# HBioquant/DiffBindFR

Hardware: AMD Instinct MI355X
Metric: poses_per_sec (higher is better)
Workload: dtype f32

## Files before the change

diffbindfr_amd/csrc/api.cpp:

```cpp
#include <cmath>
#include <cstdio>
#include <cstring>
#include <algorithm>
#include <atomic>
#include <map>

#include "common.h"

void launch_conv(const ConvArgs& a, hipStream_t st);
void launch_conv_layer(const ConvArgs* c4, hipStream_t st);
void launch_conv2(const Conv2Args& a, hipStream_t st);
void launch_conv2h(const Conv2Args& a, hipStream_t st);
void launch_convz(const ConvZArgs& a, hipStream_t st);
void launch_reduce_ln(const float* msg, const int* row_start, const int* row_cnt, int N, int D, const LNDesc& ln,
                      const float* old, int D_old, float* out, int ldo, int mode, hipStream_t st, const uint8_t* first = nullptr, unsigned long long sc_lanes = 0);
struct ReduceLayerArgs {
  const float* msg[4]; const int* row_start[4]; const int* row_cnt[4]; LNDesc ln[4];
  int NL, NA, D, D_old;
  const float* old_l; const float* old_a; float* out_l; float* out_a;
  const uint8_t* first[4]; unsigned long long sc_lanes[4];
};
static unsigned long long convz_sc_lanes(const ConvZ& z) {
  unsigned long long m = 0;
  for (int i = 0; i < z.n_io; ++i) m |= 0xfffull << (z.out_off[i] / 4);
// ... 509 lines not shown
          const PathDesc* p = pidx >= 0 ? pairs[pidx].paths[pi] : lp;
          for (int r = 0; r < 4; ++r) {
            rows_orig.push_back(pidx >= 0 ? p->w_off + (u0 + r) * p->mulo + pairs[pidx].w : -1);
            rows_scale.push_back(pidx >= 0 ? p->fold : 0.f);
          }
        }
    }
  }
  const int n_tiles = (int)rows_orig.size() / 16;
  std::vector<float> w2q((size_t)n_tiles * KT * 64 * 4), b2q((size_t)n_tiles * 16);
  for (int t = 0; t < n_tiles; ++t) {
    for (int i = 0; i < 16; ++i) { const int ro = rows_orig[16 * t + i]; b2q[16 * t + i] = ro >= 0 ? rows_scale[16 * t + i] * B2[ro] : 0.f; }
    for (int s4 = 0; s4 < KT; ++s4)
      for (int lane = 0; lane < 64; ++lane) {
        const int ro = rows_orig[16 * t + (lane & 15)];
        const float sc = rows_scale[16 * t + (lane & 15)];
        for (int q = 0; q < 4; ++q)
          w2q[(((size_t)t * KT + s4) * 64 + lane) * 4 + q] = ro >= 0 ? sc * W2[(size_t)ro * K + 16 * s4 + 4 * (lane >> 4) + q] : 0.f;
      }
  }
  memset(o, 0, sizeof *o);
  o->D_in = sp.D_in; o->D_out = sp.D_out; o->n_tiles = n_tiles; o->n_runs = (int)runs.size();
  o->W1p = base.W1p; o->b1 = base.b1;
  if (!vector_only) {
  o->W2q = upload(m, w2q, &rc);
  o->b2q = upload(m, b2q, &rc);
  }
  {
    const int rowscale = getenv("DBFR_F16_ROWSCALE") ? atoi(getenv("DBFR_F16_ROWSCALE")) : 1;
    std::vector<uint16_t> w2h((size_t)n_tiles * (CH_TILE_BYTES_HOST / 2) + 512, 0);
    std::vector<float> w2rinv((size_t)std::max(n_tiles, 1) * 16, 1.f);
    int depth_max = 0, depth_run = 0;
    for (int pass = 0; pass < 2; ++pass) {
      const bool rowf = pass == 1;
      if (rowf && !(rowscale == 2 || (rowscale == 1 && depth_max > F16_ROW_DEPTH_OK))) break;
      if (rowf) depth_run = depth_max;
      depth_max = 0;
      for (RunDesc& rd : runs) {
        const int tile0 = rd.tile0_n & 0xfffff, nt = rd.tile0_n >> 20;
        int depth = 0;
        const int k = pack_f16_tiles(w2q.data(), b2q.data(), tile0, nt, w2h.data(), &depth, rowf ? w2rinv.data() : nullptr);
        depth_max = std::max(depth_max, depth);
        rd.meta = (rd.meta & 0x00ffffffu) | ((uint32_t)(k & 0xff) << 24);
      }
      if (!rowf) depth_run = depth_max;
      else o->W2rinv = upload(m, w2rinv, &rc);
    }
    o->W2h = upload(m, w2h, &rc);
    const float* W1 = need(tm, name + ".fc.lin.0.weight", (int64_t)K * K, &rc);
    const float* B1 = need(tm, name + ".fc.lin.0.bias", K, &rc);
    if (rc) return rc;
    std::vector<float> w1q((size_t)KT * KT * 256);
    for (int mt = 0; mt < KT; ++mt)
      for (int s4 = 0; s4 < KT; ++s4)
        for (int lane = 0; lane < 64; ++lane)
          for (int q = 0; q < 4; ++q)
            w1q[(((size_t)mt * KT + s4) * 64 + lane) * 4 + q] = W1[(size_t)(16 * mt + (lane & 15)) * K + 16 * s4 + 4 * (lane >> 4) + q];
    std::vector<uint16_t> w1h((size_t)KT * (CH_TILE_BYTES_HOST / 2) + 512, 0);
    int depth1 = 0;
    o->k1 = pack_f16_tiles(w1q.data(), B1, 0, KT, w1h.data(), &depth1);
    depth_run = std::max(depth_run, depth1);
    if (rowscale == 2 || (rowscale == 1 && depth1 > F16_ROW_DEPTH_OK)) {
      std::vector<float> w1rinv((size_t)KT * 16, 1.f);
      o->k1 = pack_f16_tiles(w1q.data(), B1, 0, KT, w1h.data(), &depth1, w1rinv.data());
      o->W1rinv = upload(m, w1rinv, &rc);
    }
    o->W1h = upload(m, w1h, &rc);
    o->f16_depth = std::max(depth_max, depth1);
    o->f16_depth_run = depth_run;
  }
  o->runs = upload(m, runs, &rc);
  const int n_g = (int)groups.size();
  int total_tiles = 0;
  for (int t : group_tiles) total_tiles += t;
  for (int si = 0; si < 4; ++si) {
    const int S = 1 << si;
    int gi = 0, acc = 0;
    for (int p = 0; p < S; ++p) {
      o->part_run[si][p] = gi < n_g ? group_run0[gi] : (int)runs.size();
      const long target = (long)total_tiles * (p + 1) / S;
      while (gi < n_g && (acc + group_tiles[gi] / 2 < target || p == S - 1)) { acc += group_tiles[gi]; ++gi; }
    }
    for (int p = S; p <= 8; ++p) o->part_run[si][p] = (int)runs.size();
  }
  return rc;
}

static int pack_convz(dbfr_model* m, const TMap& tm, const std::string& name, int kind, const ConvW2& base, ConvZ* o) {
  ConvSpec sp = make_conv_spec(kind);
  const int K = sp.K;
  memset(o, 0, sizeof *o);
  if (K != 144) return fail(DBFR_ERR_ARG, "k_convz is for the K=144 convs");
  int rc = 0;
  const float* W2 = need(tm, name + ".fc.lin.3.weight", (int64_t)sp.W * K, &rc);
  const float* B2 = need(tm, name + ".fc.lin.3.bias", sp.W, &rc);
  if (rc) return rc;
  struct Col { const PathDesc* p; int u; };
  std::vector<std::vector<Col>> cols;
  std::vector<int> ios;
  for (int io = 0; io < (int)sp.out.size(); ++io) {
    if (sp.out[io].l != 0) continue;
    if (sp.out[io].mul != NS) return fail(DBFR_ERR_ARG, "scalar output irrep with a multiplicity other than 48 in " + name);
    std::vector<Col> c;
    for (int pass = 0; pass < 2; ++pass)
      for (auto& p : sp.paths) {
        if (p.io != io || p.l1 != pass) continue;
        if (p.l1 != p.l2 || p.lo != 0 || p.l1 > 1) return fail(DBFR_ERR_ARG, "unsupported scalar-output path in " + name);
        for (int u = 0; u < p.mul1; ++u) c.push_back({&p, u});
      }
    int n_scalar = 0;
    for (auto& q : c) n_scalar += q.p->l1 == 0;
    if (n_scalar % 16) return fail(DBFR_ERR_ARG, "scalar-input columns do not fill whole tiles in " + name);
    while (c.size() % 16) c.push_back({nullptr, 0});
    cols.push_back(c);
    ios.push_back(io);
  }
  if (ios.size() > 2) return fail(DBFR_ERR_ARG, "more than two scalar output irreps in " + name);
  o->n_io = (int)ios.size();
  int nct_total = 0;
  for (int i = 0; i < o->n_io; ++i) {
    o->nct[i] = (int)cols[i].size() / 16;
    for (auto& q : cols[i]) o->nc_valid[i] += q.p != nullptr;
    o->ct0[i] = nct_total;
    nct_total += o->nct[i];
    int off = 0;
    for (int j = 0; j < ios[i]; ++j) off += sp.out[j].mul * sp.out[j].dim();
    o->out_off[i] = off;
  }
  if (nct_total > CZ_MAXCT) return fail(DBFR_ERR_ARG, "too many c tiles in " + name);
  std::vector<uint32_t> cdesc((size_t)std::max(nct_total, 1) * 16, 0u);
  std::vector<float> rowinv((size_t)std::max(o->n_io, 1) * NS, 1.f);
  std::vector<uint16_t> w2z((size_t)nct_total * CZ_NKT * 8 * (CZ_TILE_BYTES / 2) + 512, 0);
  auto h16 = [](float v) { const _Float16 h = (_Float16)v; uint16_t u; memcpy(&u, &h, 2); return u; };
  for (int i = 0; i < o->n_io; ++i) {
    const auto& c = cols[i];
    for (size_t j = 0; j < c.size(); ++j)
      if (c[j].p) cdesc[(size_t)o->ct0[i] * 16 + j] = (uint32_t)(c[j].p->in_off + c[j].u * (2 * c[j].p->l1 + 1)) | ((uint32_t)c[j].p->l1 << 12) |
                                                      ((uint32_t)c[j].p->sh_off << 16) | 0x80000000u;
    auto wval = [&](int cc, int k, int w) -> float {
      if (cc >= (int)c.size() || !c[cc].p || k > K) return 0.f;
      const PathDesc* p = c[cc].p;
      const size_t row = (size_t)p->w_off + (size_t)c[cc].u * p->mulo + w;
      return p->fold * (k < K ? W2[row * K + k] : B2[row]);
    };
    for (int w = 0; w < NS; ++w) {
      float mx = 0.f;
      for (int cc = 0; cc < (int)c.size(); ++cc)
        for (int k = 0; k <= K; ++k) mx = std::max(mx, fabsf(wval(cc, k, w)));
      int s = 0;
      if (mx > 0.f) { int e = 0; (void)frexpf(mx, &e); s = std::max(-100, std::min(100, 15 - e)); }
      rowinv[(size_t)i * NS + w] = ldexpf(1.f, -s);
      const float sc = ldexpf(1.f, s);
      const int wt = w >> 4, np = w & 15;
      for (int ct = 0; ct < o->nct[i]; ++ct)
        for (int kt = 0; kt < CZ_NKT; ++kt)
          for (int v = 0; v < 8; ++v)
            for (int gp = 0; gp < 4; ++gp)
              for (int t = 0; t < 8; ++t) {
                const float val = wval(16 * ct + 4 * gp + (t & 3), 16 * kt + v + 8 * (t >> 2), w) * sc;
                const _Float16 hi = (_Float16)val;
                const size_t tile = ((size_t)(o->ct0[i] + ct) * CZ_NKT + kt) * 8 + v;
                const size_t base_h = tile * (CZ_TILE_BYTES / 2) + (size_t)(wt * 2) * 512 + (size_t)(16 * gp + np) * 8 + t;
                w2z[base_h] = h16(val);
                w2z[base_h + 512] = h16(val - (float)hi);
              }
    }
// ... 967 lines not shown
```

diffbindfr_amd/csrc/common.h:

```cpp
#pragma once
#include <hip/hip_runtime.h>
#include <stdint.h>
#include <string.h>
#include <string>
#include <vector>

#include "../../include/dbfr.h"

#define NS 48
#define NV 12
#define SH_LD 9
#define EMB 32
#define MAXD 168
#define EDGE_CHUNK 64
int dbfr_edge_chunks(int max_na, int max_nl);

enum PathType { PT_SS = 0, PT_SV = 1, PT_VS = 2, PT_VVS = 3, PT_VVV = 4, PT_VTV = 5 };

struct Irr { int mul, l, p; int dim() const { return 2 * l + 1; } };

struct PathDesc {
  int i1, i2, io, l1, l2, lo, mul1, mulo, w_off;
  float coeff;
  int type;
  int in_off, sh_off, out_off;
  float fold;
};

struct ConvSpec {
  std::vector<Irr> in, sh, out;
  std::vector<PathDesc> paths;
  int K;
  int W;
  int D_in, D_out;
};

ConvSpec make_conv_spec(int kind);
void wigner3j_real(int l1, int l2, int l3, std::vector<double>& out);
int so3_selftest(std::string& err);

struct LNDesc {
  int nblk;
  int mul[4], dim[4], off[4], is0e[4];
  const float* mean_shift;
  const float* weight;
  const float* bias;
};

struct RunDesc {
  uint32_t tile0_n;
  uint32_t meta;
  uint32_t x_off4;
  uint32_t o_off4;
};

struct ConvW {
  int K, D_in, D_out, n_tiles, W;
  int wave_tile0[5];
  const float* W1p;
  const float* b1;
  const float* W2p;
  const float* b2p;
  const RunDesc* runs;
  int wave_run0[5];
  LNDesc ln;
};

struct ConvW2 {
  int D_in, D_out, n_tiles, n_runs;
  const float* W1p;
  const float* b1;
  const float* W2q;
  const float* b2q;
  const void* W1h;
  int k1;
  int f16_depth;
  int f16_depth_run;
  const float* W2rinv;
  const float* W1rinv;
  const void* W2h;
  const RunDesc* runs;
  int part_run[4][9];
};

struct Conv2Desc {
  const int* n_edges; int max_edges;
  const int* gth;
  const float* emb;
  const float* sh;
  const float* tab1; int ld1; const int* idx1;
  const float* tab2; int ld2; const int* idx2;
  const float* x; int ldx;
  ConvW2 w;
  float* msg;
};

struct Conv2Args {
  Conv2Desc c[4];
  int n_conv;
  int* queue;
  int run_barrier, no_split;
  int skew;
  unsigned long long* trace;
};
#define C2_TRACE_CAP 4096

#define CZ_NKT 10
#define CZ_MAXCT 12
#define CZ_MAXSEG 4
#define CZ_TILE_BYTES 6144
struct ConvZ {
  int n_io;
  int nct[2];
  int ct0[2];
  int out_off[2];
  int nc_valid[2];
  const uint32_t* cdesc;
  const void* W2z;
  const float* rowinv;
  const void* W1h; int k1;
  const float* W1rinv;
};
struct ConvZDesc {
  const int* n_edges; int max_edges;
  const int* tgt;
  const int* gth;
  const float* emb; const float* sh;
  const float* tab1; int ld1; const int* idx1;
  const float* tab2; int ld2; const int* idx2;
  const float* x; int ldx;
  ConvZ w;
  float* msg; int D_out;
  const int* chunk_es;
  const int* chunk_gl;
  const int* n_chunks;
  int max_chunks;
  const float* xmax;
};
struct ConvZArgs { ConvZDesc c[4]; int n_conv; float* dbg; double* executed; int dbg_sel; };

static inline uint16_t dbfr_bf16_rne(float x) {
  uint32_t u;
  memcpy(&u, &x, 4);
  u += 0x7fffu + ((u >> 16) & 1u);
  return (uint16_t)(u >> 16);
}
static inline float dbfr_bf16_to_f32(uint16_t b) {
  const uint32_t u = (uint32_t)b << 16;
  float f;
  memcpy(&f, &u, 4);
  return f;
}

struct Mlp2 {
  int in, hid, out;
  const float* w0t;
  const float* b0;
  const float* w1t;
  const float* b1;
};

struct EdgeSet {
  int cap;
  int* n_edges;
  int* tgt;
// ... 47 lines not shown
```

diffbindfr_amd/csrc/conv2h.hip:

```cpp
#include <cstdio>
#include <cstdlib>
#include <type_traits>

#include "common.h"

typedef float f32x4 __attribute__((ext_vector_type(4)));
typedef float f32x2 __attribute__((ext_vector_type(2)));
typedef _Float16 f16x8 __attribute__((ext_vector_type(8)));
typedef _Float16 f16x4 __attribute__((ext_vector_type(4)));
typedef _Float16 f16x2 __attribute__((ext_vector_type(2)));
typedef unsigned u32x4 __attribute__((ext_vector_type(4)));
typedef unsigned u32x2 __attribute__((ext_vector_type(2)));

#define CH_TILE_BYTES 9280
#define CH_TAIL_OFF 8192
#define CH_BIAS_OFF 9216
#define CH_RING_BYTES 10240

__device__ __forceinline__ void split2x2(float x0, float x1, unsigned& hi, unsigned& lo) {
  const f16x2 h = __builtin_convertvector((f32x2){x0, x1}, f16x2);
  const f16x2 l = __builtin_convertvector((f32x2){x0 - (float)h[0], x1 - (float)h[1]}, f16x2);
  hi = __builtin_bit_cast(unsigned, h);
  lo = __builtin_bit_cast(unsigned, l);
}

__device__ __forceinline__ void scale4(f32x4& o, const f32x4& v, float s) { o[0] = v[0] * s; o[1] = v[1] * s; o[2] = v[2] * s; o[3] = v[3] * s; }
__device__ __forceinline__ void sum4(f32x4& o, const f32x4& a, const f32x4& b) { o[0] = a[0] + b[0]; o[1] = a[1] + b[1]; o[2] = a[2] + b[2]; o[3] = a[3] + b[3]; }

#define C2_XLD 124
#define C2_WAVE_FLOATS (32 * C2_XLD + 32 * 10 + 32 * 8 + 32)

template <int NW, int ABL = 0>
__global__ __launch_bounds__(64 * NW, 2) void k_conv2h(Conv2Args a) {
  constexpr int K = 144, KT = 9;
  constexpr bool ROWF = (ABL & 1024) != 0;
  constexpr int EPB = 32 * NW;
  extern __shared__ __attribute__((aligned(16))) float lds[];
  const int tid = threadIdx.x, lane = tid & 63, wave = tid >> 6;
  const int n = lane & 15, g = lane >> 4;
  if (wave >= NW / 2) __builtin_amdgcn_s_setprio(1);
  const char* ring = reinterpret_cast<const char*>(lds);
  float* xs = lds + CH_RING_BYTES / 4 + wave * C2_WAVE_FLOATS;
  float* shs = xs + 32 * C2_XLD;
  float* ms = shs + 32 * 10;
  int* s_gth = reinterpret_cast<int*>(ms + 32 * 8);

  if (a.trace && blockIdx.x == 0 && tid == 0) { a.trace[0] = __builtin_readcyclecounter(); a.trace[1] = __builtin_amdgcn_s_memrealtime(); }
  int nb0 = 0, nb1 = 0, nb2 = 0, nb3 = 0;
  {
    auto blocks = [&](int c) { return c < a.n_conv ? (min(*a.c[c].n_edges, a.c[c].max_edges) + EPB - 1) / EPB : 0; };
    nb0 = blocks(0); nb1 = blocks(1); nb2 = blocks(2); nb3 = blocks(3);
  }
  const int N = nb0 + nb1 + nb2 + nb3;
  const int n_wg = gridDim.x;
  const int full = (N / n_wg) * n_wg, rem = N - full;
  int si = 0;
  if (rem > 0 && !a.no_split) {
    int best = 0x7fffffff;
#pragma unroll
    for (int c = 0; c < 4; ++c) {
      const int cost = (((rem << c) + n_wg - 1) / n_wg) * ((128 >> c) + 6);
      if (cost < best) { best = cost; si = c; }
    }
  }
  const int total = full + (rem << si);

  for (int it = 0;; ++it) {
    asm volatile("s_waitcnt vmcnt(0) lgkmcnt(0)" ::: "memory");
    __syncthreads();
    const int u = (int)blockIdx.x + it * n_wg;
    if (u >= total) break;
    int blk, part = 0, psi = 0;
    if (u < full) blk = u;
    else { const int v = u - full; blk = full + (v >> si); part = v & ((1 << si) - 1); psi = si; }
    int c = 0;
    if (blk >= nb0) { blk -= nb0; c = 1; if (blk >= nb1) { blk -= nb1; c = 2; if (blk >= nb2) { blk -= nb2; c = 3; } } }
    const Conv2Desc& d = a.c[c];
    const int E = min(*d.n_edges, d.max_edges);
    const int e0 = blk * EPB + 32 * wave;
    const int D_in = d.w.D_in, D_out = d.w.D_out;
    const int vW = lane * 16, vB = g * 16;
    const int wv = __builtin_amdgcn_readfirstlane(wave);
    const int r_begin = d.w.part_run[psi][part], r_end = d.w.part_run[psi][part + 1];
    int t_last = 0, t_first = 0;
    if (r_begin < r_end) {
      const RunDesc rl = d.w.runs[r_end - 1];
      t_last = (rl.tile0_n & 0xfffff) + (rl.tile0_n >> 20) - 1;
      t_first = d.w.runs[r_begin].tile0_n & 0xfffff;
    }
    const __amdgpu_buffer_rsrc_t rW = __builtin_amdgcn_make_buffer_rsrc((void*)d.w.W2h, 0, d.w.n_tiles * CH_TILE_BYTES, 0x00020000);
    const int shA = wv & 7, shB = wv % 6;
    const int offA = shA < 6 ? ((shA / 3) * 4 + shA % 3) * 1024 : CH_BIAS_OFF;
    const int offB = shB < 4 ? ((shB >> 1) * 4 + 3) * 1024 + (shB & 1) * 512 : CH_TAIL_OFF + (shB - 4) * 512;
    const int vA = (shA < 6 || lane < 4) ? lane * 16 : 0x40000000;
    char* ringw = const_cast<char*>(ring);
    u32x4 stgA = {0u, 0u, 0u, 0u};
    u32x2 stgB = {0u, 0u};
    auto fetchA = [&](int tile) { if (!(ABL & (4 | 16))) stgA = __builtin_bit_cast(u32x4, __builtin_amdgcn_raw_buffer_load_b128(rW, vA, ((ABL & 512) ? (tile & 7) : tile) * CH_TILE_BYTES + offA, 0)); };
    auto fetchB = [&](int tile) { if (!(ABL & (4 | 16))) stgB = __builtin_bit_cast(u32x2, __builtin_amdgcn_raw_buffer_load_b64(rW, lane * 8, ((ABL & 512) ? (tile & 7) : tile) * CH_TILE_BYTES + offB, 0)); };
    auto putA = [&] { if (!(ABL & (4 | 8))) *reinterpret_cast<u32x4*>(ringw + offA + vW) = stgA; };
    auto putB = [&] { if (!(ABL & (4 | 8))) *reinterpret_cast<u32x2*>(ringw + offB + lane * 8) = stgB; };
    using I0 = std::integral_constant<int, 0>; using I1 = std::integral_constant<int, 1>;
    using I2 = std::integral_constant<int, 2>; using I3 = std::integral_constant<int, 3>;
    if (r_begin < r_end) {
      fetchA(t_first); fetchB(t_first);
    }

    int ev[2], gthv[2];
    const float* r0[2]; const float* r1[2]; const float* r2[2];
#pragma unroll
    for (int b = 0; b < 2; ++b) {
      const int e = e0 + 16 * b + n;
      ev[b] = min(e, E - 1);
      gthv[b] = d.gth[ev[b]];
      r0[b] = d.emb + (size_t)ev[b] * NS;
      r1[b] = d.tab1 + (size_t)d.idx1[ev[b]] * d.ld1;
      r2[b] = d.tab2 + (size_t)d.idx2[ev[b]] * d.ld2;
    }
    if (g == 0) { s_gth[n] = gthv[0]; s_gth[16 + n] = gthv[1]; }
    if (lane < 32) {
      const int e = min(e0 + lane, E - 1);
      const float* sp = d.sh + (size_t)e * SH_LD;
      float s[9];
#pragma unroll
      for (int k = 0; k < 9; ++k) { s[k] = sp[k]; shs[lane * 10 + k] = s[k]; }
      const float r3 = 1.7320508075688772f;
      float* m = ms + lane * 8;
      m[0] = -s[6] - r3 * s[8]; m[1] = r3 * s[5]; m[2] = r3 * s[4]; m[3] = 2.f * s[6]; m[4] = r3 * s[7]; m[5] = -s[6] + r3 * s[8];
    }
    u32x4 Bh[2][2][4];
    u32x4 Btc[2];
    float se[2], ue[2];
    {
      const __amdgpu_buffer_rsrc_t rW1 = __builtin_amdgcn_make_buffer_rsrc((void*)d.w.W1h, 0, KT * CH_TILE_BYTES, 0x00020000);
      u32x4 Ah[2][2][4];
      u32x4 Atc[2];
      float sa[2];
      int ja[2];
#pragma unroll
      for (int b = 0; b < 2; ++b) {
        f32x4 Ba[KT];
        float amx = 0.f;
#pragma unroll
        for (int s4 = 0; s4 < KT; ++s4) {
          const float* src = s4 < 3 ? r0[b] : s4 < 6 ? r1[b] : r2[b];
          Ba[s4] = *reinterpret_cast<const f32x4*>(src + 16 * (s4 % 3) + 4 * g);
#pragma unroll
          for (int q = 0; q < 4; ++q) amx = fmaxf(amx, fabsf(Ba[s4][q]));
        }
        amx = fmaxf(amx, __shfl_xor(amx, 16));
        amx = fmaxf(amx, __shfl_xor(amx, 32));
        ja[b] = max(-14, __builtin_amdgcn_frexp_expf(amx));
        sa[b] = __builtin_amdgcn_ldexpf(1.f, 15 - ja[b]);
#pragma unroll
        for (int s4 = 0; s4 < KT; ++s4) {
          unsigned hi0, lo0, hi1, lo1;
          split2x2(Ba[s4][0] * sa[b], Ba[s4][1] * sa[b], hi0, lo0);
          split2x2(Ba[s4][2] * sa[b], Ba[s4][3] * sa[b], hi1, lo1);
          if (s4 < 8) {
            Ah[b][0][s4 >> 1][2 * (s4 & 1)] = hi0; Ah[b][0][s4 >> 1][2 * (s4 & 1) + 1] = hi1;
            Ah[b][1][s4 >> 1][2 * (s4 & 1)] = lo0; Ah[b][1][s4 >> 1][2 * (s4 & 1) + 1] = lo1;
          } else {
            Atc[b] = (u32x4){lo0, lo1, hi0, hi1};
          }
        }
      }
      constexpr int NST = KT * 4;
      u32x4 F[3][2];
      u32x4 Ft;
      f32x4 bb;
      auto ld_step = [&](int i, u32x4 (&f)[2]) {
#pragma unroll
        for (int p = 0; p < 2; ++p) f[p] = __builtin_bit_cast(u32x4, __builtin_amdgcn_raw_buffer_load_b128(rW1, vW, (i >> 2) * CH_TILE_BYTES + (p * 4 + (i & 3)) * 1024, 0));
      };
      auto ld_tail = [&](int m) {
        Ft = __builtin_bit_cast(u32x4, __builtin_amdgcn_raw_buffer_load_b128(rW1, vW, m * CH_TILE_BYTES + CH_TAIL_OFF, 0));
        bb = __builtin_bit_cast(f32x4, __builtin_amdgcn_raw_buffer_load_b128(rW1, vB, m * CH_TILE_BYTES + CH_BIAS_OFF, 0));
      };
      ld_step(0, F[0]); ld_step(1, F[1]); ld_tail(0);
      float H[2][KT][4];
      float mx[2] = {0.f, 0.f};
      const f32x4 zero = {0.f, 0.f, 0.f, 0.f};
#define AHB(b, p, s) __builtin_bit_cast(f16x8, Ah[b][p][s])
#define FW(i, p) __builtin_bit_cast(f16x8, F[(i) % 3][p])
#pragma unroll
      for (int m = 0; m < KT; ++m) {
        f32x4 aS[2], aB[2];
        scale4(aS[0], bb, sa[0]); scale4(aS[1], bb, sa[1]);
        aB[0] = zero; aB[1] = zero;
#pragma unroll
        for (int s = 0; s < 4; ++s) {
          const int i = m * 4 + s;
          aS[0] = __builtin_amdgcn_mfma_f32_16x16x32_f16(FW(i, 0), AHB(0, 1, s), aS[0], 0, 0, 0);
          aS[1] = __builtin_amdgcn_mfma_f32_16x16x32_f16(FW(i, 0), AHB(1, 1, s), aS[1], 0, 0, 0);
          aS[0] = __builtin_amdgcn_mfma_f32_16x16x32_f16(FW(i, 1), AHB(0, 0, s), aS[0], 0, 0, 0);
          aS[1] = __builtin_amdgcn_mfma_f32_16x16x32_f16(FW(i, 1), AHB(1, 0, s), aS[1], 0, 0, 0);
          aB[0] = __builtin_amdgcn_mfma_f32_16x16x32_f16(FW(i, 0), AHB(0, 0, s), aB[0], 0, 0, 0);
          aB[1] = __builtin_amdgcn_mfma_f32_16x16x32_f16(FW(i, 0), AHB(1, 0, s), aB[1], 0, 0, 0);
          __builtin_amdgcn_sched_barrier(0);
          if (i + 2 < NST) ld_step(i + 2, F[(i + 2) % 3]);
        }
        {
          const f16x8 fw = __builtin_bit_cast(f16x8, Ft);
          const f16x4 fh = __builtin_bit_cast(f16x4, (u32x2){Ft[0], Ft[1]});
          aS[0] = __builtin_amdgcn_mfma_f32_16x16x32_f16(fw, __builtin_bit_cast(f16x8, Atc[0]), aS[0], 0, 0, 0);
          aS[1] = __builtin_amdgcn_mfma_f32_16x16x32_f16(fw, __builtin_bit_cast(f16x8, Atc[1]), aS[1], 0, 0, 0);
          aB[0] = __builtin_amdgcn_mfma_f32_16x16x16f16(fh, __builtin_bit_cast(f16x4, (u32x2){Atc[0][2], Atc[0][3]}), aB[0], 0, 0, 0);
          aB[1] = __builtin_amdgcn_mfma_f32_16x16x16f16(fh, __builtin_bit_cast(f16x4, (u32x2){Atc[1][2], Atc[1][3]}), aB[1], 0, 0, 0);
          __builtin_amdgcn_sched_barrier(0);
          if (m + 1 < KT) ld_tail(m + 1);
        }
        f32x4 rv = {1.f, 1.f, 1.f, 1.f};
        if constexpr (ROWF) if (d.w.W1rinv) rv = *reinterpret_cast<const f32x4*>(d.w.W1rinv + 16 * m + 4 * g);
#pragma unroll
        for (int b = 0; b < 2; ++b)
#pragma unroll
          for (int r = 0; r < 4; ++r) { H[b][m][r] = fmaxf(aS[b][r] + aB[b][r], 0.f); if constexpr (ROWF) H[b][m][r] *= rv[r]; mx[b] = fmaxf(mx[b], H[b][m][r]); }
      }
#undef AHB
#undef FW
      const int k1 = d.w.k1;
#pragma unroll
      for (int b = 0; b < 2; ++b) {
        float m2 = fmaxf(mx[b], __shfl_xor(mx[b], 16));
        m2 = fmaxf(m2, __shfl_xor(m2, 32));
        const int j = __builtin_amdgcn_frexp_expf(m2);
        const int tot = max(-120, min(64, 15 - j + k1 + 15 - ja[b]));
        const float t = __builtin_amdgcn_ldexpf(1.f, tot - k1 - 15 + ja[b]);
        se[b] = __builtin_amdgcn_ldexpf(1.f, tot);
        ue[b] = __builtin_amdgcn_ldexpf(1.f, -tot);
#pragma unroll
        for (int m = 0; m < KT; ++m) {
          unsigned hi0, lo0, hi1, lo1;
          split2x2(H[b][m][0] * t, H[b][m][1] * t, hi0, lo0);
          split2x2(H[b][m][2] * t, H[b][m][3] * t, hi1, lo1);
          if (m < 8) {
            Bh[b][0][m >> 1][2 * (m & 1)] = hi0; Bh[b][0][m >> 1][2 * (m & 1) + 1] = hi1;
            Bh[b][1][m >> 1][2 * (m & 1)] = lo0; Bh[b][1][m >> 1][2 * (m & 1) + 1] = lo1;
          } else {
            Btc[b] = (u32x4){lo0, lo1, hi0, hi1};
          }
        }
      }
    }
    __builtin_amdgcn_wave_barrier();
    {
      const int d4 = min(D_in, 120) >> 2;
      const float* xsrc = d.x + (size_t)s_gth[lane & 31] * d.ldx;
      float* xdst = xs + (lane & 31) * C2_XLD;
      f32x4 v[15];
#pragma unroll
      for (int j = 0; j < 15; ++j) v[j] = *reinterpret_cast<const f32x4*>(xsrc + 4 * min(2 * j + (lane >> 5), d4 - 1));
#pragma unroll
      for (int j = 0; j < 15; ++j) *reinterpret_cast<f32x4*>(xdst + 4 * min(2 * j + (lane >> 5), d4 - 1)) = v[j];
    }
    __builtin_amdgcn_wave_barrier();

    if (ABL & 64) {
      asm volatile("" ::"v"(Bh[0][0][0]), "v"(Bh[1][1][3]), "v"(Btc[1]));
      continue;
    }
    float oacc[2][3];
#pragma unroll
    for (int b = 0; b < 2; ++b) oacc[b][0] = oacc[b][1] = oacc[b][2] = 0.f;
    const float* xs_lane = xs + n * C2_XLD;
    const float* sh_lane = shs + n * 10;
    f16x8 FA[2], FB[2];
    f16x8 FT;
    f32x4 bias_n;
    f32x4 accN[2];
    f32x4 accS[2], accB[2];
    f32x4 accp[2];
    f32x4 rinv_c = {1.f, 1.f, 1.f, 1.f}, rinv_n = {1.f, 1.f, 1.f, 1.f};
    const float* rinv_base = ROWF && d.w.W2rinv ? d.w.W2rinv + 4 * g : nullptr;
    auto sumr4 = [&](f32x4& o, const f32x4& x, const f32x4& y) {
      if constexpr (ROWF) { o[0] = (x[0] + y[0]) * rinv_c[0]; o[1] = (x[1] + y[1]) * rinv_c[1]; o[2] = (x[2] + y[2]) * rinv_c[2]; o[3] = (x[3] + y[3]) * rinv_c[3]; }
      else sum4(o, x, y);
    };
    auto rd_step = [&](auto jc, f16x8 (&F)[2]) {
      constexpr int j = decltype(jc)::value;
#pragma unroll
      for (int i = 0; i < 2; ++i) F[i] = *reinterpret_cast<const f16x8*>(ring + (i * 4 + j) * 1024 + vW);
    };
    auto ring_barrier = [&] {
      __builtin_amdgcn_sched_barrier(0);
      asm volatile("s_waitcnt lgkmcnt(0)" ::: "memory");
      if (!(ABL & 2)) __builtin_amdgcn_s_barrier();
      __builtin_amdgcn_sched_barrier(0);
    };
#define HB(b, p, s) __builtin_bit_cast(f16x8, Bh[b][p][s])
#define M32(C, wp, b, hp, F, s) __builtin_amdgcn_mfma_f32_16x16x32_f16(F[wp], HB(b, hp, s), C, 0, 0, 0)
#define MT32(C, b) __builtin_amdgcn_mfma_f32_16x16x32_f16(FT, __builtin_bit_cast(f16x8, Btc[b]), C, 0, 0, 0)
#define MT16(C, b) __builtin_amdgcn_mfma_f32_16x16x16f16(__builtin_shufflevector(FT, FT, 0, 1, 2, 3), __builtin_bit_cast(f16x4, (u32x2){Btc[b][2], Btc[b][3]}), C, 0, 0, 0)
#define SLOT(m) do { op(std::integral_constant<int, (m)>{}); __builtin_amdgcn_sched_barrier(0); } while (0)
    auto tile = [&](int t, auto&& op) {
      const f32x4 zero = {0.f, 0.f, 0.f, 0.f};
      accS[0] = M32(accN[0], 0, 0, 1, FA, 0); if (ABL & 256) putB(); SLOT(0);
      accS[1] = M32(accN[1], 0, 1, 1, FA, 0); if (ABL & 256) fetchB(min(t + 1, t_last)); SLOT(1);
      accS[0] = M32(accS[0], 1, 0, 0, FA, 0); rd_step(I1{}, FB); SLOT(2);
      accS[1] = M32(accS[1], 1, 1, 0, FA, 0); SLOT(3);
      accB[0] = M32(zero, 0, 0, 0, FA, 0); SLOT(4);
      accB[1] = M32(zero, 0, 1, 0, FA, 0); SLOT(5);
      accS[0] = M32(accS[0], 0, 0, 1, FB, 1); SLOT(6);
      accS[1] = M32(accS[1], 0, 1, 1, FB, 1); SLOT(7);
      accS[0] = M32(accS[0], 1, 0, 0, FB, 1); rd_step(I2{}, FA); SLOT(8);
      accS[1] = M32(accS[1], 1, 1, 0, FB, 1); if (!(ABL & 256)) putB(); SLOT(9);
      accB[0] = M32(accB[0], 0, 0, 0, FB, 1); if (!(ABL & (256 | 32))) fetchB(min(t + 1, t_last)); SLOT(10);
      accB[1] = M32(accB[1], 0, 1, 0, FB, 1); SLOT(11);
      ring_barrier();
      accS[0] = M32(accS[0], 0, 0, 1, FA, 2); if (ABL & 256) putA(); SLOT(12);
      accS[1] = M32(accS[1], 0, 1, 1, FA, 2); if (ABL & 256) fetchA(min(t + 2, t_last)); SLOT(13);
      accS[0] = M32(accS[0], 1, 0, 0, FA, 2); rd_step(I3{}, FB); SLOT(14);
      accS[1] = M32(accS[1], 1, 1, 0, FA, 2); SLOT(15);
      accB[0] = M32(accB[0], 0, 0, 0, FA, 2); SLOT(16);
      accB[1] = M32(accB[1], 0, 1, 0, FA, 2); SLOT(17);
      accS[0] = M32(accS[0], 0, 0, 1, FB, 3); SLOT(18);
      accS[1] = M32(accS[1], 0, 1, 1, FB, 3); SLOT(19);
      accS[0] = M32(accS[0], 1, 0, 0, FB, 3); FT = *reinterpret_cast<const f16x8*>(ring + CH_TAIL_OFF + vW);
      if constexpr (ROWF) if (rinv_base) rinv_n = *reinterpret_cast<const f32x4*>(rinv_base + 16 * min(t + 1, t_last));
      SLOT(20);
      accS[1] = M32(accS[1], 1, 1, 0, FB, 3); if (!(ABL & 256)) putA(); SLOT(21);
      accB[0] = M32(accB[0], 0, 0, 0, FB, 3); if (!(ABL & (256 | 32))) fetchA(min(t + 2, t_last)); SLOT(22);
      accB[1] = M32(accB[1], 0, 1, 0, FB, 3); SLOT(23);
      ring_barrier();
      accS[0] = MT32(accS[0], 0); bias_n = *reinterpret_cast<const f32x4*>(ring + CH_BIAS_OFF + vB); SLOT(24);
      accB[0] = MT16(accB[0], 0); rd_step(I0{}, FA); SLOT(25);
      accS[1] = MT32(accS[1], 1); SLOT(26);
      accB[1] = MT16(accB[1], 1); SLOT(27);
      sumr4(accp[1], accS[1], accB[1]);
      if constexpr (ROWF) rinv_c = rinv_n;
      __builtin_amdgcn_sched_barrier(0);
    };
#undef SLOT
    int x_phase = 0;
    if (r_begin < r_end) {
      putA();
      fetchA(min(t_first + 1, t_last));
      asm volatile("s_waitcnt lgkmcnt(0)" ::: "memory");
      __builtin_amdgcn_s_barrier();
      rd_step(I0{}, FA);
      bias_n = *reinterpret_cast<const f32x4*>(ring + CH_BIAS_OFF + vB);
      scale4(accN[0], bias_n, se[0]); scale4(accN[1], bias_n, se[1]);
      if constexpr (ROWF) if (rinv_base) rinv_c = *reinterpret_cast<const f32x4*>(rinv_base + 16 * t_first);
    }
    for (int r = r_begin; r < r_end; ++r) {
      const RunDesc rd = d.w.runs[r];
      const int tile0 = rd.tile0_n & 0xfffff, nt = rd.tile0_n >> 20;
      const int type = rd.meta & 15, flags = (rd.meta >> 4) & 3, sh_off = (rd.meta >> 8) & 15, x_step = (rd.meta >> 12) & 0xff;
      const int xph = (rd.meta >> 20) & 1;
      const float run_inv = __builtin_amdgcn_ldexpf(1.f, -((int)rd.meta >> 24));
      const int xo = (rd.x_off4 >> (8 * g)) & 0xff, oo = (rd.o_off4 >> (8 * g)) & 0xff;
      if (xph != x_phase) {
        __builtin_amdgcn_wave_barrier();
        {
          const float* xsrc = d.x + (size_t)s_gth[lane & 31] * d.ldx + 120;
          float* xdst = xs + (lane & 31) * C2_XLD;
          f32x4 v[6];
#pragma unroll
          for (int j = 0; j < 6; ++j) v[j] = *reinterpret_cast<const f32x4*>(xsrc + 4 * (2 * j + (lane >> 5)));
#pragma unroll
          for (int j = 0; j < 6; ++j) *reinterpret_cast<f32x4*>(xdst + 4 * (2 * j + (lane >> 5))) = v[j];
        }
        __builtin_amdgcn_wave_barrier();
        x_phase = xph;
      }
      if (flags & 1) {
#pragma unroll
        for (int b = 0; b < 2; ++b) oacc[b][0] = oacc[b][1] = oacc[b][2] = 0.f;
      }
      auto run = [&](auto type_c) {
        constexpr int TYPE = decltype(type_c)::value;
        constexpr bool VIN = !(TYPE == PT_SS || TYPE == PT_SV);
        constexpr bool VOUT = !(TYPE == PT_SS || TYPE == PT_VVS);
        constexpr int NSV = (TYPE == PT_SS || TYPE == PT_VS) ? 1 : (TYPE == PT_VTV ? 0 : 3);
        float S[2][NSV ? NSV : 1];
        float Mv[2][TYPE == PT_VTV ? 6 : 1];
#pragma unroll
        for (int b = 0; b < 2; ++b) {
          if (TYPE != PT_VTV) {
            const float* sp = sh_lane + 160 * b + sh_off;
#pragma unroll
            for (int k = 0; k < NSV; ++k) S[b][k] = sp[k] * run_inv;
          } else {
            const float* mp = ms + (16 * b + n) * 8;
#pragma unroll
            for (int k = 0; k < 6; ++k) Mv[b][k] = mp[k] * run_inv;
          }
        }
        f32x4 cxa, cxb, cxc;
        float czr[2][3] = {{0.f, 0.f, 0.f}, {0.f, 0.f, 0.f}};
        auto cop = [&](auto bc, auto kc, const float* xp) {
          constexpr int b = decltype(bc)::value;
          constexpr int K = decltype(kc)::value;
          if (ABL & 1) { if (K == 1) asm volatile("" ::"v"(accp[b])); return; }
          const f32x4 v = accp[b];
          const f32x4* x4 = reinterpret_cast<const f32x4*>(xp + 16 * b * C2_XLD);
          if (VIN && K == 2) cxb = x4[1];
          if (VIN && K == 6) cxc = x4[2];
          if (K == 0) cxa = x4[0];
          if (!VIN) {
            if (K == 1) czr[b][0] += v[0] * cxa[0];
            if (K == 2) czr[b][0] += v[1] * cxa[1];
            if (K == 3) czr[b][0] += v[2] * cxa[2];
            if (K == 4) czr[b][0] += v[3] * cxa[3];
          } else {
            if (K == 1) czr[b][0] += v[0] * cxa[0];
            if (K == 2) czr[b][1] += v[0] * cxa[1];
            if (K == 3) czr[b][2] += v[0] * cxa[2];
            if (K == 4) czr[b][0] += v[1] * cxa[3];
            if (K == 5) czr[b][1] += v[1] * cxb[0];
            if (K == 6) czr[b][2] += v[1] * cxb[1];
            if (K == 7) czr[b][0] += v[2] * cxb[2];
            if (K == 8) czr[b][1] += v[2] * cxb[3];
            if (K == 9) czr[b][2] += v[2] * cxc[0];
            if (K == 10) czr[b][0] += v[3] * cxc[1];
            if (K == 11) czr[b][1] += v[3] * cxc[2];
            if (K == 12) czr[b][2] += v[3] * cxc[3];
          }
        };
        auto finish = [&](auto bc) {
          constexpr int b = decltype(bc)::value;
          if (ABL & 1) return;
          const float cz0 = czr[b][0], cz1 = czr[b][1], cz2 = czr[b][2];
          if (TYPE == PT_SS) oacc[b][0] += cz0 * S[b][0];
          else if (TYPE == PT_SV) { oacc[b][0] += cz0 * S[b][0]; oacc[b][1] += cz0 * S[b][1]; oacc[b][2] += cz0 * S[b][2]; }
          else if (TYPE == PT_VS) { oacc[b][0] += cz0 * S[b][0]; oacc[b][1] += cz1 * S[b][0]; oacc[b][2] += cz2 * S[b][0]; }
          else if (TYPE == PT_VVS) { oacc[b][0] += cz0 * S[b][0]; oacc[b][0] += cz1 * S[b][1]; oacc[b][0] += cz2 * S[b][2]; }
          else if (TYPE == PT_VVV) {
            oacc[b][0] += cz1 * S[b][2]; oacc[b][1] += cz2 * S[b][0]; oacc[b][2] += cz0 * S[b][1];
            oacc[b][0] -= cz2 * S[b][1]; oacc[b][1] -= cz0 * S[b][2]; oacc[b][2] -= cz1 * S[b][0];
          } else {
            oacc[b][0] += Mv[b][0] * cz0; oacc[b][1] += Mv[b][1] * cz0; oacc[b][2] += Mv[b][2] * cz0;
            oacc[b][0] += Mv[b][1] * cz1; oacc[b][1] += Mv[b][3] * cz1; oacc[b][2] += Mv[b][4] * cz1;
            oacc[b][0] += Mv[b][2] * cz2; oacc[b][1] += Mv[b][4] * cz2; oacc[b][2] += Mv[b][5] * cz2;
          }
        };
        using B0 = std::integral_constant<int, 0>;
        using B1 = std::integral_constant<int, 1>;
        auto travel = [&](auto mc, const float* xp) {
          constexpr int m = decltype(mc)::value;
          if constexpr (m == 0) cop(B0{}, std::integral_constant<int, 0>{}, xp);
          if constexpr (m >= 3 && m <= 14) cop(B0{}, std::integral_constant<int, m - 2>{}, xp);
          if constexpr (m == 12) cop(B1{}, std::integral_constant<int, 0>{}, xp);
          if constexpr (m >= 15 && m <= 26) cop(B1{}, std::integral_constant<int, m - 14>{}, xp);
          if constexpr (m == 26) scale4(accN[0], bias_n, se[0]);
          if constexpr (m == 27) { scale4(accN[1], bias_n, se[1]); sumr4(accp[0], accS[0], accB[0]); }
        };
        const float* xp = xs_lane + xo;
        accp[0] = (f32x4){0.f, 0.f, 0.f, 0.f}; accp[1] = (f32x4){0.f, 0.f, 0.f, 0.f};
        for (int i = 0; i < nt; ++i) {
          tile(tile0 + i, [&](auto mc) { travel(mc, xp); });
          if (i) xp += x_step;
        }
        __builtin_amdgcn_sched_barrier(0);
#define COPS(b) cop(b, std::integral_constant<int, 0>{}, xp); cop(b, std::integral_constant<int, 1>{}, xp); cop(b, std::integral_constant<int, 2>{}, xp); \
        cop(b, std::integral_constant<int, 3>{}, xp); cop(b, std::integral_constant<int, 4>{}, xp); cop(b, std::integral_constant<int, 5>{}, xp); \
        cop(b, std::integral_constant<int, 6>{}, xp); cop(b, std::integral_constant<int, 7>{}, xp); cop(b, std::integral_constant<int, 8>{}, xp); \
        cop(b, std::integral_constant<int, 9>{}, xp); cop(b, std::integral_constant<int, 10>{}, xp); cop(b, std::integral_constant<int, 11>{}, xp); \
        cop(b, std::integral_constant<int, 12>{}, xp); finish(b);
        COPS(B0{}) COPS(B1{})
#undef COPS
        if (flags & 2) {
          if (oo < D_out) {
#pragma unroll
            for (int b = 0; b < 2; ++b)
              if (e0 + 16 * b + n < E) {
                float* op = d.msg + (size_t)(e0 + 16 * b + n) * D_out + oo;
                op[0] = oacc[b][0] * ue[b];
                if (VOUT) { op[1] = oacc[b][1] * ue[b]; op[2] = oacc[b][2] * ue[b]; }
              }
          }
        }
      };
      switch (type) {
        case PT_SS: run(std::integral_constant<int, PT_SS>{}); break;
        case PT_SV: run(std::integral_constant<int, PT_SV>{}); break;
        case PT_VS: run(std::integral_constant<int, PT_VS>{}); break;
        case PT_VVS: run(std::integral_constant<int, PT_VVS>{}); break;
        case PT_VVV: run(std::integral_constant<int, PT_VVV>{}); break;
        default: run(std::integral_constant<int, PT_VTV>{}); break;
      }
    }
#undef M32
#undef MT32
#undef MT16
#undef HB
#undef TB
  }
  if (a.trace && blockIdx.x == 0 && tid == 0) { a.trace[2] = __builtin_readcyclecounter(); a.trace[3] = __builtin_amdgcn_s_memrealtime(); }
}

void launch_conv2h(const Conv2Args& a, hipStream_t st) {
  static int no_split = getenv("DBFR_CONV2_NOSPLIT") ? atoi(getenv("DBFR_CONV2_NOSPLIT")) : 0;
  constexpr int NW = 8;
  const size_t lds = CH_RING_BYTES + (size_t)NW * C2_WAVE_FLOATS * sizeof(float);
  const int n_cu = dbfr_current_cu_count();
  Conv2Args b = a;
  b.skew = 0;
  b.run_barrier = 0;
  b.no_split = no_split;
#define V(x) { if (dbfr_launch_check(hipFuncSetAttribute(reinterpret_cast<const void*>(&k_conv2h<NW, x>), hipFuncAttributeMaxDynamicSharedMemorySize, (int)lds), "k_conv2h: hipFuncSetAttribute(MaxDynamicSharedMemorySize)")) return; \
               hipLaunchKernelGGL((k_conv2h<NW, x>), dim3(n_cu), dim3(64 * NW), lds, st, b); return; }
#ifdef DBFR_DEV_VARIANTS
  static int abl = getenv("DBFR_CONV2H_ABL") ? atoi(getenv("DBFR_CONV2H_ABL")) : 0;
  if (abl == 1) V(1) if (abl == 2) V(2) if (abl == 3) V(3) if (abl == 4) V(4) if (abl == 7) V(7) if (abl == 8) V(8) if (abl == 16) V(16)
  if (abl == 32) V(32) if (abl == 64) V(64) if (abl == 256) V(256) if (abl == 512) V(512)
#endif
  for (int i = 0; i < a.n_conv; ++i)
    if (a.c[i].w.W2rinv || a.c[i].w.W1rinv) V(1024)
  V(0)
#undef V
}
```

Baseline: 510.9.

## Hoist edge loads and W1 weight prefetch ahead of the first conv2h layer

Reorders the prologue of the conv2h kernel so that edge embeddings, tables and SH values are loaded early. The first W1 weight steps, bias, tail and row-inverse are prefetched before the tab1/tab2 gathers, giving the memory latency room to overlap. Per-part first and last tile indices are precomputed on the host into a new part_tile table, which avoids dependent loads of run descriptors. Edge counts are read once per block through readfirstlane. Register pressure rises from the larger prefetch arrays, and optional timing stamps are added behind a dev macro.

```diff
diff --git a/diffbindfr_amd/csrc/api.cpp b/diffbindfr_amd/csrc/api.cpp
--- a/diffbindfr_amd/csrc/api.cpp
+++ b/diffbindfr_amd/csrc/api.cpp
@@ -615,6 +615,13 @@
       while (gi < n_g && (acc + group_tiles[gi] / 2 < target || p == S - 1)) { acc += group_tiles[gi]; ++gi; }
     }
     for (int p = S; p <= 8; ++p) o->part_run[si][p] = (int)runs.size();
+    for (int p = 0; p < 8; ++p) {
+      const int r0 = o->part_run[si][p], r1 = o->part_run[si][p + 1];
+      if (r0 >= r1) continue;
+      const uint32_t t_first = runs[r0].tile0_n & 0xfffff, t_last = (runs[r1 - 1].tile0_n & 0xfffff) + (runs[r1 - 1].tile0_n >> 20) - 1;
+      if (t_last >= (1u << 16)) return fail(DBFR_ERR_ARG, "conv too large for the part tile table");
+      o->part_tile[si][p] = t_first | (t_last << 16);
+    }
   }
   return rc;
 }
diff --git a/diffbindfr_amd/csrc/common.h b/diffbindfr_amd/csrc/common.h
--- a/diffbindfr_amd/csrc/common.h
+++ b/diffbindfr_amd/csrc/common.h
@@ -81,6 +81,7 @@
   const void* W2h;
   const RunDesc* runs;
   int part_run[4][9];
+  uint32_t part_tile[4][8];
 };
 
 struct Conv2Desc {
diff --git a/diffbindfr_amd/csrc/conv2h.hip b/diffbindfr_amd/csrc/conv2h.hip
--- a/diffbindfr_amd/csrc/conv2h.hip
+++ b/diffbindfr_amd/csrc/conv2h.hip
@@ -27,6 +27,20 @@
 __device__ __forceinline__ void scale4(f32x4& o, const f32x4& v, float s) { o[0] = v[0] * s; o[1] = v[1] * s; o[2] = v[2] * s; o[3] = v[3] * s; }
 __device__ __forceinline__ void sum4(f32x4& o, const f32x4& a, const f32x4& b) { o[0] = a[0] + b[0]; o[1] = a[1] + b[1]; o[2] = a[2] + b[2]; o[3] = a[3] + b[3]; }
 
+#ifdef DBFR_DEV_VARIANTS
+#define C2H_STAMP(k) do { __builtin_amdgcn_sched_barrier(0); stamp[k] = __builtin_readcyclecounter(); __builtin_amdgcn_sched_barrier(0); } while (0)
+#define C2H_STAMPS_OUT() do { if (a.trace && blockIdx.x == 0 && tid == 0 && it < 64) { for (int k = 0; k < 4; ++k) a.trace[8 + 4 * it + k] = stamp[k]; } } while (0)
+#else
+#define C2H_STAMP(k) do { } while (0)
+#define C2H_STAMPS_OUT() do { } while (0)
+#endif
+
+#ifndef C2H_RING_DEPTH
+#define C2H_RING_DEPTH 2
+#endif
+#ifndef C2H_PIN
+#define C2H_PIN 0
+#endif
 #define C2_XLD 124
 #define C2_WAVE_FLOATS (32 * C2_XLD + 32 * 10 + 32 * 8 + 32)
 
@@ -46,11 +60,9 @@
   int* s_gth = reinterpret_cast<int*>(ms + 32 * 8);
 
   if (a.trace && blockIdx.x == 0 && tid == 0) { a.trace[0] = __builtin_readcyclecounter(); a.trace[1] = __builtin_amdgcn_s_memrealtime(); }
-  int nb0 = 0, nb1 = 0, nb2 = 0, nb3 = 0;
-  {
-    auto blocks = [&](int c) { return c < a.n_conv ? (min(*a.c[c].n_edges, a.c[c].max_edges) + EPB - 1) / EPB : 0; };
-    nb0 = blocks(0); nb1 = blocks(1); nb2 = blocks(2); nb3 = blocks(3);
-  }
+  auto edges = [&](int c) { return c < a.n_conv ? __builtin_amdgcn_readfirstlane(min(*a.c[c].n_edges, a.c[c].max_edges)) : 0; };
+  const int E0 = edges(0), E1 = edges(1), E2 = edges(2), E3 = edges(3);
+  const int nb0 = (E0 + EPB - 1) / EPB, nb1 = (E1 + EPB - 1) / EPB, nb2 = (E2 + EPB - 1) / EPB, nb3 = (E3 + EPB - 1) / EPB;
   const int N = nb0 + nb1 + nb2 + nb3;
   const int n_wg = gridDim.x;
   const int full = (N / n_wg) * n_wg, rem = N - full;
@@ -70,24 +82,26 @@
     __syncthreads();
     const int u = (int)blockIdx.x + it * n_wg;
     if (u >= total) break;
+#ifdef DBFR_DEV_VARIANTS
+    unsigned long long stamp[4] = {0ull, 0ull, 0ull, 0ull};
+#endif
+    C2H_STAMP(0);
     int blk, part = 0, psi = 0;
     if (u < full) blk = u;
     else { const int v = u - full; blk = full + (v >> si); part = v & ((1 << si) - 1); psi = si; }
     int c = 0;
     if (blk >= nb0) { blk -= nb0; c = 1; if (blk >= nb1) { blk -= nb1; c = 2; if (blk >= nb2) { blk -= nb2; c = 3; } } }
     const Conv2Desc& d = a.c[c];
-    const int E = min(*d.n_edges, d.max_edges);
+    int cs = c;
+    asm volatile("" : "+s"(cs));
+    const int E = cs == 0 ? E0 : cs == 1 ? E1 : cs == 2 ? E2 : E3;
     const int e0 = blk * EPB + 32 * wave;
     const int D_in = d.w.D_in, D_out = d.w.D_out;
     const int vW = lane * 16, vB = g * 16;
     const int wv = __builtin_amdgcn_readfirstlane(wave);
     const int r_begin = d.w.part_run[psi][part], r_end = d.w.part_run[psi][part + 1];
-    int t_last = 0, t_first = 0;
-    if (r_begin < r_end) {
-      const RunDesc rl = d.w.runs[r_end - 1];
-      t_last = (rl.tile0_n & 0xfffff) + (rl.tile0_n >> 20) - 1;
-      t_first = d.w.runs[r_begin].tile0_n & 0xfffff;
-    }
+    const unsigned pt = d.w.part_tile[psi][part];
+    const int t_first = pt & 0xffff, t_last = pt >> 16;
     const __amdgpu_buffer_rsrc_t rW = __builtin_amdgcn_make_buffer_rsrc((void*)d.w.W2h, 0, d.w.n_tiles * CH_TILE_BYTES, 0x00020000);
     const int shA = wv & 7, shB = wv % 6;
     const int offA = shA < 6 ? ((shA / 3) * 4 + shA % 3) * 1024 : CH_BIAS_OFF;
@@ -102,52 +116,83 @@
     auto putB = [&] { if (!(ABL & (4 | 8))) *reinterpret_cast<u32x2*>(ringw + offB + lane * 8) = stgB; };
     using I0 = std::integral_constant<int, 0>; using I1 = std::integral_constant<int, 1>;
     using I2 = std::integral_constant<int, 2>; using I3 = std::integral_constant<int, 3>;
-    if (r_begin < r_end) {
-      fetchA(t_first); fetchB(t_first);
-    }
-
-    int ev[2], gthv[2];
-    const float* r0[2]; const float* r1[2]; const float* r2[2];
+    int ev[2], gthv[2], i1v[2], i2v[2];
 #pragma unroll
     for (int b = 0; b < 2; ++b) {
       const int e = e0 + 16 * b + n;
       ev[b] = min(e, E - 1);
       gthv[b] = d.gth[ev[b]];
-      r0[b] = d.emb + (size_t)ev[b] * NS;
-      r1[b] = d.tab1 + (size_t)d.idx1[ev[b]] * d.ld1;
-      r2[b] = d.tab2 + (size_t)d.idx2[ev[b]] * d.ld2;
-    }
-    if (g == 0) { s_gth[n] = gthv[0]; s_gth[16 + n] = gthv[1]; }
-    if (lane < 32) {
-      const int e = min(e0 + lane, E - 1);
-      const float* sp = d.sh + (size_t)e * SH_LD;
-      float s[9];
-#pragma unroll
-      for (int k = 0; k < 9; ++k) { s[k] = sp[k]; shs[lane * 10 + k] = s[k]; }
+      i1v[b] = d.idx1[ev[b]];
+      i2v[b] = d.idx2[ev[b]];
+    }
+    __builtin_amdgcn_sched_barrier(0);
+    f32x4 Ba[2][9];
+#pragma unroll
+    for (int b = 0; b < 2; ++b) {
+      const float* r0 = d.emb + (size_t)ev[b] * NS;
+#pragma unroll
+      for (int s4 = 0; s4 < 3; ++s4) Ba[b][s4] = *reinterpret_cast<const f32x4*>(r0 + 16 * s4 + 4 * g);
+    }
+    float shv[9];
+    {
+      const float* sp = d.sh + (size_t)min(e0 + (lane & 31), E - 1) * SH_LD;
+#pragma unroll
+      for (int k = 0; k < 9; ++k) shv[k] = sp[k];
+    }
+    fetchA(t_first); fetchB(t_first);
+    constexpr int RD = C2H_RING_DEPTH;
+    const __amdgpu_buffer_rsrc_t rW1 = __builtin_amdgcn_make_buffer_rsrc((void*)d.w.W1h, 0, KT * CH_TILE_BYTES, 0x00020000);
+    u32x4 F[RD + 1][2];
+    u32x4 Ft;
+    f32x4 bb;
+    auto ld_step = [&](int i, u32x4 (&f)[2]) {
+#pragma unroll
+      for (int p = 0; p < 2; ++p) f[p] = __builtin_bit_cast(u32x4, __builtin_amdgcn_raw_buffer_load_b128(rW1, vW, (i >> 2) * CH_TILE_BYTES + (p * 4 + (i & 3)) * 1024, 0));
+    };
+    auto ld_tail = [&](int m) { Ft = __builtin_bit_cast(u32x4, __builtin_amdgcn_raw_buffer_load_b128(rW1, vW, m * CH_TILE_BYTES + CH_TAIL_OFF, 0)); };
+    auto ld_bias = [&](int m) { bb = __builtin_bit_cast(f32x4, __builtin_amdgcn_raw_buffer_load_b128(rW1, vB, m * CH_TILE_BYTES + CH_BIAS_OFF, 0)); };
+    ld_bias(0); ld_tail(0);
+    const bool has_rv = ROWF && d.w.W1rinv != nullptr;
+    const __amdgpu_buffer_rsrc_t rRV = __builtin_amdgcn_make_buffer_rsrc((void*)d.w.W1rinv, 0, has_rv ? K * 4 : 0, 0x00020000);
+    f32x4 rvl = {0.f, 0.f, 0.f, 0.f};
+    auto ld_rv = [&](int m) { if constexpr (ROWF) rvl = __builtin_bit_cast(f32x4, __builtin_amdgcn_raw_buffer_load_b128(rRV, vB, m * 64, 0)); };
+    ld_rv(0);
+#pragma unroll
+    for (int i = 0; i < RD; ++i) ld_step(i, F[i]);
+    __builtin_amdgcn_sched_barrier(0);
+#pragma unroll
+    for (int b = 0; b < 2; ++b) {
+      const float* r1 = d.tab1 + (size_t)i1v[b] * d.ld1;
+      const float* r2 = d.tab2 + (size_t)i2v[b] * d.ld2;
+#pragma unroll
+      for (int s4 = 0; s4 < 3; ++s4) Ba[b][3 + s4] = *reinterpret_cast<const f32x4*>(r1 + 16 * s4 + 4 * g);
+#pragma unroll
+      for (int s4 = 0; s4 < 3; ++s4) Ba[b][6 + s4] = *reinterpret_cast<const f32x4*>(r2 + 16 * s4 + 4 * g);
+    }
+    __builtin_amdgcn_sched_barrier(0);
+    s_gth[n] = gthv[0]; s_gth[16 + n] = gthv[1];
+    {
+#pragma unroll
+      for (int k = 0; k < 9; ++k) shs[(lane & 31) * 10 + k] = shv[k];
       const float r3 = 1.7320508075688772f;
-      float* m = ms + lane * 8;
-      m[0] = -s[6] - r3 * s[8]; m[1] = r3 * s[5]; m[2] = r3 * s[4]; m[3] = 2.f * s[6]; m[4] = r3 * s[7]; m[5] = -s[6] + r3 * s[8];
+      float* m = ms + (lane & 31) * 8;
+      m[0] = -shv[6] - r3 * shv[8]; m[1] = r3 * shv[5]; m[2] = r3 * shv[4]; m[3] = 2.f * shv[6]; m[4] = r3 * shv[7]; m[5] = -shv[6] + r3 * shv[8];
     }
     u32x4 Bh[2][2][4];
     u32x4 Btc[2];
     float se[2], ue[2];
     {
-      const __amdgpu_buffer_rsrc_t rW1 = __builtin_amdgcn_make_buffer_rsrc((void*)d.w.W1h, 0, KT * CH_TILE_BYTES, 0x00020000);
       u32x4 Ah[2][2][4];
       u32x4 Atc[2];
       float sa[2];
       int ja[2];
 #pragma unroll
       for (int b = 0; b < 2; ++b) {
-        f32x4 Ba[KT];
         float amx = 0.f;
 #pragma unroll
-        for (int s4 = 0; s4 < KT; ++s4) {
-          const float* src = s4 < 3 ? r0[b] : s4 < 6 ? r1[b] : r2[b];
-          Ba[s4] = *reinterpret_cast<const f32x4*>(src + 16 * (s4 % 3) + 4 * g);
-#pragma unroll
-          for (int q = 0; q < 4; ++q) amx = fmaxf(amx, fabsf(Ba[s4][q]));
-        }
+        for (int s4 = 0; s4 < KT; ++s4)
+#pragma unroll
+          for (int q = 0; q < 4; ++q) amx = fmaxf(amx, fabsf(Ba[b][s4][q]));
         amx = fmaxf(amx, __shfl_xor(amx, 16));
         amx = fmaxf(amx, __shfl_xor(amx, 32));
         ja[b] = max(-14, __builtin_amdgcn_frexp_expf(amx));
@@ -155,8 +200,8 @@
 #pragma unroll
         for (int s4 = 0; s4 < KT; ++s4) {
           unsigned hi0, lo0, hi1, lo1;
-          split2x2(Ba[s4][0] * sa[b], Ba[s4][1] * sa[b], hi0, lo0);
-          split2x2(Ba[s4][2] * sa[b], Ba[s4][3] * sa[b], hi1, lo1);
+          split2x2(Ba[b][s4][0] * sa[b], Ba[b][s4][1] * sa[b], hi0, lo0);
+          split2x2(Ba[b][s4][2] * sa[b], Ba[b][s4][3] * sa[b], hi1, lo1);
           if (s4 < 8) {
             Ah[b][0][s4 >> 1][2 * (s4 & 1)] = hi0; Ah[b][0][s4 >> 1][2 * (s4 & 1) + 1] = hi1;
             Ah[b][1][s4 >> 1][2 * (s4 & 1)] = lo0; Ah[b][1][s4 >> 1][2 * (s4 & 1) + 1] = lo1;
@@ -166,23 +211,12 @@
         }
       }
       constexpr int NST = KT * 4;
-      u32x4 F[3][2];
-      u32x4 Ft;
-      f32x4 bb;
-      auto ld_step = [&](int i, u32x4 (&f)[2]) {
-#pragma unroll
-        for (int p = 0; p < 2; ++p) f[p] = __builtin_bit_cast(u32x4, __builtin_amdgcn_raw_buffer_load_b128(rW1, vW, (i >> 2) * CH_TILE_BYTES + (p * 4 + (i & 3)) * 1024, 0));
-      };
-      auto ld_tail = [&](int m) {
-        Ft = __builtin_bit_cast(u32x4, __builtin_amdgcn_raw_buffer_load_b128(rW1, vW, m * CH_TILE_BYTES + CH_TAIL_OFF, 0));
-        bb = __builtin_bit_cast(f32x4, __builtin_amdgcn_raw_buffer_load_b128(rW1, vB, m * CH_TILE_BYTES + CH_BIAS_OFF, 0));
-      };
-      ld_step(0, F[0]); ld_step(1, F[1]); ld_tail(0);
       float H[2][KT][4];
       float mx[2] = {0.f, 0.f};
       const f32x4 zero = {0.f, 0.f, 0.f, 0.f};
+      C2H_STAMP(1);
 #define AHB(b, p, s) __builtin_bit_cast(f16x8, Ah[b][p][s])
-#define FW(i, p) __builtin_bit_cast(f16x8, F[(i) % 3][p])
+#define FW(i, p) __builtin_bit_cast(f16x8, F[(i) % (RD + 1)][p])
 #pragma unroll
       for (int m = 0; m < KT; ++m) {
         f32x4 aS[2], aB[2];
@@ -198,7 +232,9 @@
           aB[0] = __builtin_amdgcn_mfma_f32_16x16x32_f16(FW(i, 0), AHB(0, 0, s), aB[0], 0, 0, 0);
           aB[1] = __builtin_amdgcn_mfma_f32_16x16x32_f16(FW(i, 0), AHB(1, 0, s), aB[1], 0, 0, 0);
           __builtin_amdgcn_sched_barrier(0);
-          if (i + 2 < NST) ld_step(i + 2, F[(i + 2) % 3]);
+          if (i + RD < NST) ld_step(i + RD, F[(i + RD) % (RD + 1)]);
+          if (s == 0 && m + 1 < KT) ld_bias(m + 1);
+          if (C2H_PIN) __builtin_amdgcn_sched_barrier(0);
         }
         {
           const f16x8 fw = __builtin_bit_cast(f16x8, Ft);
@@ -209,16 +245,19 @@
           aB[1] = __builtin_amdgcn_mfma_f32_16x16x16f16(fh, __builtin_bit_cast(f16x4, (u32x2){Atc[1][2], Atc[1][3]}), aB[1], 0, 0, 0);
           __builtin_amdgcn_sched_barrier(0);
           if (m + 1 < KT) ld_tail(m + 1);
+          if (C2H_PIN) __builtin_amdgcn_sched_barrier(0);
         }
         f32x4 rv = {1.f, 1.f, 1.f, 1.f};
-        if constexpr (ROWF) if (d.w.W1rinv) rv = *reinterpret_cast<const f32x4*>(d.w.W1rinv + 16 * m + 4 * g);
+        if constexpr (ROWF) { rv[0] = has_rv ? rvl[0] : 1.f; rv[1] = has_rv ? rvl[1] : 1.f; rv[2] = has_rv ? rvl[2] : 1.f; rv[3] = has_rv ? rvl[3] : 1.f; }
 #pragma unroll
         for (int b = 0; b < 2; ++b)
 #pragma unroll
           for (int r = 0; r < 4; ++r) { H[b][m][r] = fmaxf(aS[b][r] + aB[b][r], 0.f); if constexpr (ROWF) H[b][m][r] *= rv[r]; mx[b] = fmaxf(mx[b], H[b][m][r]); }
+        if constexpr (ROWF) if (m + 1 < KT) { __builtin_amdgcn_sched_barrier(0); ld_rv(m + 1); __builtin_amdgcn_sched_barrier(0); }
       }
 #undef AHB
 #undef FW
+      C2H_STAMP(2);
       const int k1 = d.w.k1;
 #pragma unroll
       for (int b = 0; b < 2; ++b) {
@@ -258,6 +297,7 @@
 
     if (ABL & 64) {
       asm volatile("" ::"v"(Bh[0][0][0]), "v"(Bh[1][1][3]), "v"(Btc[1]));
+      C2H_STAMPS_OUT();
       continue;
     }
     float oacc[2][3];
@@ -338,6 +378,7 @@
       fetchA(min(t_first + 1, t_last));
       asm volatile("s_waitcnt lgkmcnt(0)" ::: "memory");
       __builtin_amdgcn_s_barrier();
+      C2H_STAMP(3);
       rd_step(I0{}, FA);
       bias_n = *reinterpret_cast<const f32x4*>(ring + CH_BIAS_OFF + vB);
       scale4(accN[0], bias_n, se[0]); scale4(accN[1], bias_n, se[1]);
@@ -481,6 +522,7 @@
         default: run(std::integral_constant<int, PT_VTV>{}); break;
       }
     }
+    C2H_STAMPS_OUT();
 #undef M32
 #undef MT32
 #undef MT16
```

Measured after the change: 488.5. -4.4%, worse.
